# danshapero/sigma

Hardware: AMD Instinct MI355X
Metric: SpMV GB/s (achieved HBM) + CG iters/sec on 5-pt Laplacian, N=1e7 (higher is better)
Workload: dtype f64; 1 GPU; 5-point 2D Poisson CSR, 3162x3162 rows per GPU (rank 0: n=9998244, nnz=49978572), fp64 SpMV y=A*x; rows_per_gpu=9998244, nnz_per_gpu=49978572, parallelism=row-partition x1, matrix_resident_bytes_per_gpu=479920788, reference_layout_bytes_per_gpu=639735844, full=False

## Files before the change

sigma_amd/csrc/sgm_internal.hpp:

```cpp
#pragma once
#include <hip/hip_runtime.h>

#include <cstdarg>
#include <cstdint>
#include <cstdio>
#include <cstring>
#include <string>
#include <atomic>
#include <utility>
#include <vector>

#include "../../include/sigma_hip.h"

namespace sgm {

extern std::string g_err;
int fail(int code, const char *fmt, ...);

#define SGM_HIP(call)                                                              \
    do {                                                                           \
        hipError_t e__ = (call);                                                   \
        if (e__ != hipSuccess)                                                     \
            return sgm::fail(SGM_ERR_HIP, "%s:%d: %s -> %s", __FILE__, __LINE__,   \
                             #call, hipGetErrorString(e__));                       \
// ... 115 lines not shown
};

struct SliceSched { int32_t *tab = nullptr; int32_t lo = 0, hi = 0, grid = 0, iters = 0, band = 0; };

struct Part {
    MatOptions opt = g_opt.mat;
    int32_t n = 0;
    int32_t ncol_own = 0;
    int32_t n_halo = 0;
    int32_t int_lo = 0, int_hi = 0;
    int64_t nnz = 0;
    int64_t row_begin = 0;
    int32_t *rowptr = nullptr;
    int32_t *col = nullptr;
    double *val = nullptr;
    uint8_t *code = nullptr;
    int32_t *dict = nullptr;
    int32_t ndict = 0;
    int32_t dict_reach = 0;
    int32_t max_row = 0;
    double *sval = nullptr;
    uint32_t *scode = nullptr;
    int32_t *scol = nullptr;
    uint8_t *sbcode = nullptr;
    bool lean = false;
    double *sl_val = nullptr;
    int32_t *sl_col = nullptr;
    uint16_t *sl_perm = nullptr;
    int64_t *sl_off = nullptr;
    int64_t sl_total = 0;
    int32_t *sl_win0 = nullptr;
    int32_t sl_gs = 1;
    int32_t sl_span = 0;
    int32_t sw = 0;
    int32_t sched_period = 0;
    mutable SliceSched sched[3];
    mutable int nsched = 0;
    const int32_t *run_sched = nullptr;
    int32_t run_iters = 0;
    int32_t max_d = 0;
    int32_t *ecol = nullptr;
    double *eval = nullptr;
    int32_t *edeg = nullptr;
    uint8_t *ecode = nullptr;
    int32_t emdp = 0;
    int32_t *cb_perm = nullptr;
    double *cb_sval = nullptr;
    uint16_t *cb_lcol = nullptr;
    int32_t *cb_bstart = nullptr;
    uint16_t *cb_lpos = nullptr;
    void *cb_fdesc = nullptr;
    double *cb_P = nullptr;
    int32_t cb_cols = 0, cb_nb = 0, cb_R = 0, cb_ntiles = 0, cb_chunks = 0;
    int32_t cb_maxd = 0;
    int64_t cb_count = 0;
    double col_spread = -1.0;
    std::vector<HaloNbr> nbrs;
    double *xext = nullptr;
    int dot_grid_override = 0;
    int64_t xlen() const { return (int64_t)ncol_own + n_halo; }
};

}

namespace sgm { struct AlgPlan; void alg_plan_free(AlgPlan *p); void alg_plan_rows(const AlgPlan *p, int32_t out[2]); }

// ... 258 lines not shown
```

sigma_amd/csrc/sgm_layouts.hip:

```cpp
#include "sgm_spmv_select.hpp"

namespace sgm {

__global__ void k_dec1(int32_t *a, int64_t n)
{
    int64_t i = (int64_t)blockIdx.x * blockDim.x + threadIdx.x;
    const int64_t stride = (int64_t)gridDim.x * blockDim.x;
    for (; i < n; i += stride) a[i] -= 1;
}

__global__ void k_check_ptr1(const int32_t *__restrict__ ptr1, int64_t n, int64_t nnz, unsigned long long *bad)
{
    int64_t i = (int64_t)blockIdx.x * blockDim.x + threadIdx.x;
    const int64_t stride = (int64_t)gridDim.x * blockDim.x;
    for (; i <= n; i += stride) {
        const int32_t a = ptr1[i];
        bool ok = true;
        if (i == 0) ok = a == 1;
        if (i < n) ok = ok && ptr1[i + 1] >= a;
        else ok = ok && (int64_t)a - 1 == nnz;
        if (!ok) atomicMin(bad, (unsigned long long)i);
    }
}

// ... 245 lines not shown
{
    if (!p.lean || p.val) return SGM_OK;
    SGM_TRY(dalloc(&p.val, (size_t)p.nnz + 2));
    SGM_HIP(hipMemsetAsync(p.val + p.nnz, 0, 2 * sizeof(double), g_rt.stream));
    return SGM_OK;
}
void csr_release_arrays(const Part &cp)
{
    Part &p = const_cast<Part &>(cp);
    if (!p.lean || !lean_applies(p)) return;
    (void)hipStreamSynchronize(g_rt.stream);
    dfree(p.val); dfree(p.col); dfree(p.code);
    p.val = nullptr; p.col = nullptr; p.code = nullptr;
}

int pack_sliced(Part &p)
{
    if (p.sl_val && p.n > 0) {
        const int64_t nch = (((int64_t)p.n + kSlRows - 1) / kSlRows) * (kSlRows / kSellChunk);
        hipLaunchKernelGGL(k_sell_fill, dim3((unsigned)std::min<int64_t>((nch + 3) / 4, 65536)), dim3(256), 0, g_rt.stream, p.n,
                           (const int32_t *)p.rowptr, (const int32_t *)nullptr, (const double *)p.val, (const int64_t *)p.sl_off,
                           (const uint16_t *)p.sl_perm, (int32_t *)nullptr, p.sl_val);
        SGM_HIP(hipGetLastError());
    }
    if ((!p.scode && !p.scol && !p.sbcode) || p.n == 0) return SGM_OK;
    const int64_t nsl = ((int64_t)p.n + kSlRows - 1) / kSlRows;
    if (p.ecol)
        hipLaunchKernelGGL(k_sl_pack_ell, dim3((unsigned)std::min<int64_t>(nsl, 65536)), dim3(256), 0, g_rt.stream, p.n, p.sw,
                           p.max_d, (const double *)p.eval, p.sval);
    else
        hipLaunchKernelGGL(k_sl_pack, dim3((unsigned)std::min<int64_t>(nsl, 65536)), dim3(256), 0, g_rt.stream, p.n, p.sw,
                           (const int32_t *)p.rowptr, (const double *)p.val, p.sval);
    SGM_HIP(hipGetLastError());
    return SGM_OK;
}

__global__ void k_fill32(int64_t n, int32_t *a, int32_t v)
{
    int64_t i = (int64_t)blockIdx.x * blockDim.x + threadIdx.x;
    const int64_t stride = (int64_t)gridDim.x * blockDim.x;
    for (; i < n; i += stride) a[i] = v;
}

constexpr int kDictSlots = 1024;
constexpr int32_t kDictEmpty = INT32_MIN;
__global__ __launch_bounds__(256) void k_dict_collect(int32_t n, const int32_t *__restrict__ rowptr, const int32_t *__restrict__ col,
                                                      int32_t *table, int *count, int *max_row)
{
    constexpr int kLocal = 512;
    __shared__ int32_t ltab[kLocal];
    __shared__ int lcount;
    for (int t = threadIdx.x; t < kLocal; t += 256) ltab[t] = kDictEmpty;
    if (threadIdx.x == 0) lcount = 0;
    __syncthreads();
    int mr = 0;
    int32_t mine[8];
#pragma unroll
    for (int t = 0; t < 8; ++t) mine[t] = kDictEmpty;
    int next = 0;
    for (int32_t i = blockIdx.x * blockDim.x + threadIdx.x; i < n; i += gridDim.x * blockDim.x) {
        const int32_t s0 = rowptr[i], e = rowptr[i + 1];
        mr = max(mr, e - s0);
        for (int32_t k = s0; k < e; ++k) {
            const int32_t off = col[k] - i;
            bool known = false;
#pragma unroll
// ... 448 lines not shown
        return fail(SGM_ERR_UNSUPPORTED, "clone_csr_plain: single-GPU CSR matrices only");
    const Part &p = A->parts[0];
    SGM_TRY(csr_need_arrays(p));
    struct Release { const Part &p; ~Release() { csr_release_arrays(p); } } rel{p};
    sgm_mat C = new sgm_mat_s;
    C->fmt = SGM_FMT_CSR; C->nrow = A->nrow; C->ncol = A->ncol; C->nnz = A->nnz;
    C->parts.resize(1);
    Part &q = C->parts[0];
    q.opt.csr_offset_dict = 0; q.opt.csr_sliced = 0; q.opt.csr_sell = 0; q.opt.csr_lean = 0; q.opt.slice_sched = 0;
    q.n = p.n; q.ncol_own = p.ncol_own; q.n_halo = 0; q.nnz = p.nnz; q.max_row = p.max_row;
    hipStream_t st = g_rt.stream;
    int rc = dalloc(&q.rowptr, (size_t)p.n + 1);
    if (rc == SGM_OK) rc = dalloc(&q.col, (size_t)p.nnz + 4);
    if (rc == SGM_OK) rc = dalloc(&q.val, (size_t)p.nnz + 2);
    if (rc != SGM_OK) { sgm_mat_destroy(C); return rc; }
    (void)hipMemcpyAsync(q.rowptr, p.rowptr, ((size_t)p.n + 1) * 4, hipMemcpyDeviceToDevice, st);
    (void)hipMemsetAsync(q.col + p.nnz, 0, 16, st);
    (void)hipMemsetAsync(q.val + p.nnz, 0, 16, st);
    if (p.nnz) {
        (void)hipMemcpyAsync(q.col, p.col, (size_t)p.nnz * 4, hipMemcpyDeviceToDevice, st);
        (void)hipMemcpyAsync(q.val, p.val, (size_t)p.nnz * 8, hipMemcpyDeviceToDevice, st);
    }
    if (hipStreamSynchronize(st) != hipSuccess || hipGetLastError() != hipSuccess) { sgm_mat_destroy(C); return fail(SGM_ERR_HIP, "clone_csr_plain: copy failed"); }
    *out = C;
    return SGM_OK;
}

int rebuild_csr_formats(Part &p)
{
    SGM_TRY(csr_need_arrays(p));
    p.lean = false;
    dfree(p.code); dfree(p.dict); dfree(p.sval); dfree(p.scode); dfree(p.scol); dfree(p.sbcode);
    p.code = nullptr; p.dict = nullptr; p.sval = nullptr; p.scode = nullptr; p.scol = nullptr; p.sbcode = nullptr;
    free_sell(p);
    free_ell_colblock(p);
    p.ndict = 0; p.dict_reach = 0; p.sw = 0; p.max_row = 0; p.sched_period = 0;
    free_slice_sched(p);
    return build_offset_dict(p, nullptr, nullptr);
}
int rebuild_ell_formats(Part &p)
{
    dfree(p.ecode); dfree(p.dict); dfree(p.sval); dfree(p.scode);
    p.ecode = nullptr; p.dict = nullptr; p.dict_reach = 0; p.emdp = 0; p.sval = nullptr; p.scode = nullptr; p.sw = 0; p.sched_period = 0;
    free_slice_sched(p);
    SGM_TRY(build_ell_offset_dict(p));
    SGM_TRY(build_ell_colblock(p));
    return refresh_ell_colblock_values(p);
}
int sgm_invalidate_transpose(sgm_mat A)
{
    if (A->T) { sgm_mat_destroy(A->T); A->T = nullptr; }
    dfree(A->tperm);
    A->tperm = nullptr;
    A->t_stale = true;
    return SGM_OK;
}

void free_part(Part &p)
{
    dfree(p.rowptr); dfree(p.col); dfree(p.val); dfree(p.code); dfree(p.dict); dfree(p.sval); dfree(p.scode); dfree(p.scol); dfree(p.sbcode); dfree(p.ecol); dfree(p.eval); dfree(p.edeg); dfree(p.ecode); dfree(p.xext);
    for (auto &nb : p.nbrs) { dfree(nb.send_idx); dfree(nb.send_buf); }
    free_slice_sched(p);
    free_ell_colblock(p);
    free_sell(p);
    p = Part();
}

}
```

sigma_amd/csrc/sgm_mat.hip:

```cpp
#include "sgm_spmv_select.hpp"

namespace sgm {

int stage_in(Staged &s, const double *v, int64_t n, int where, bool copy)
{
    if (where == SGM_DEVICE && (reinterpret_cast<uintptr_t>(v) & 15) == 0) {
        s.dev = const_cast<double *>(v);
        return SGM_OK;
    }
    SGM_TRY(dalloc(&s.dev, (size_t)n));
    s.owned = true;
    if (copy)
        SGM_HIP(hipMemcpyAsync(s.dev, v, (size_t)n * 8,
                               where == SGM_HOST ? hipMemcpyHostToDevice : hipMemcpyDeviceToDevice,
                               g_rt.stream));
    return SGM_OK;
}
int stage_out(const Staged &s, double *v, int64_t n, int where)
{
    if (!s.owned) return SGM_OK;
    SGM_HIP(hipMemcpyAsync(v, s.dev, (size_t)n * 8,
                           where == SGM_HOST ? hipMemcpyDeviceToHost : hipMemcpyDeviceToDevice,
                           g_rt.stream));
    SGM_HIP(hipStreamSynchronize(g_rt.stream));
// ... 356 lines not shown
    return SGM_OK;
}

int sgm_mat_set_option(sgm_mat A, const char *name, int value)
{
    SGM_TRY(require_init());
    if (!A || !name) return fail(SGM_ERR_BAD_ARG, "sgm_mat_set_option: null argument");
    int v = 0;
    SGM_TRY(normalise_option(name, value, &v));
    MatOptions probe;
    if (!mat_option_field(probe, name)) return fail(SGM_ERR_BAD_ARG, "sgm_mat_set_option: '%s' is not a matrix option", name);
    if (A->fmt == SGM_FMT_COMPOSITE) {
        for (sgm_mat_s *B : A->blocks)
            if (B) SGM_TRY(sgm_mat_set_option(B, name, value));
        return SGM_OK;
    }
    const bool cb_shape = !strcmp(name, "ell_colblock_cols") || !strcmp(name, "ell_colblock_rows");
    for (Part &p : A->parts) {
        int *f = mat_option_field(p.opt, name);
        const int old = *f;
        *f = v;
        if (old == v) continue;
        if ((p.ecol || (!p.lean && p.rowptr && p.col && p.val && p.n_halo == 0 && !p.sval && !p.sl_val)) &&
            (cb_shape || (!strcmp(name, "ell_colblock") && ((old != 0) != (v != 0) || v == 2 || old == 2)))) {
            SGM_TRY(build_ell_colblock(p));
            SGM_TRY(refresh_ell_colblock_values(p));
            SGM_HIP(hipStreamSynchronize(g_rt.stream));
        }
        if (!strcmp(name, "csr_lean") && !p.ecol) {
            if (v == 0) { SGM_TRY(csr_need_arrays(p)); p.lean = false; }
            else csr_go_lean(p);
        }
        if (!strcmp(name, "slice_sched")) free_slice_sched(p);
    }
    if (A->T) SGM_TRY(sgm_mat_set_option(A->T, name, value));
    return SGM_OK;
}

int sgm_mat_matvec(sgm_mat A, const double *x, double *y, int where)
{
    return matvec_impl(A, x, y, where, false);
}

int sgm_mat_matvec_add(sgm_mat A, const double *x, double *y, int where)
{
    return matvec_impl(A, x, y, where, true);
}

int sgm_composite_create(sgm_mat *out, int32_t nrb, int32_t ncb, const int32_t *row_ptr, const int32_t *col_ptr,
                         const sgm_mat *blocks)
{
    SGM_TRY(require_init());
    if (!out || nrb < 1 || ncb < 1 || !row_ptr || !col_ptr || !blocks)
        return fail(SGM_ERR_BAD_ARG, "sgm_composite_create: bad argument");
    sgm_mat A = new sgm_mat_s;
    A->fmt = SGM_FMT_COMPOSITE;
    for (int i = 0; i <= nrb; ++i) A->blk_row_ptr.push_back(row_ptr[i] - 1);
    for (int j = 0; j <= ncb; ++j) A->blk_col_ptr.push_back(col_ptr[j] - 1);
    A->nrow = A->blk_row_ptr[nrb];
    A->ncol = A->blk_col_ptr[ncb];
    A->blocks.assign(blocks, blocks + (size_t)nrb * ncb);
    sgm_comm comm = nullptr;
    bool any_local = false;
    for (int it = 0; it < nrb; ++it)
        for (int jt = 0; jt < ncb; ++jt) {
            sgm_mat C = A->blocks[(size_t)it * ncb + jt];
// ... 142 lines not shown
    else if (use_sliced(p)) snprintf(name, len, "k_csr_sl<W=%d>", p.sw);
    else if (use_slicedb(p)) snprintf(name, len, "k_csr_slb<W=%d>", p.sw);
    else if (use_sliced32(p)) snprintf(name, len, "k_csr_sl32<W=%d>", p.sw);
    else if (use_sell(p)) snprintf(name, len, p.sl_win0 && p.opt.csr_xwindow ? "k_csr_sell<pad=%.3f,xw=%dx%d>" : "k_csr_sell<pad=%.3f>",
                                   p.nnz ? (double)p.sl_total / (double)p.nnz : 1.0, p.sl_span, p.sl_gs);
    else if (use_offset_dict(p)) snprintf(name, len, "k_csr_do<256,%d,CW=1>", do_tile_for(p));
    else if (use_row_owner(p)) snprintf(name, len, "k_csr_do<256,%d,CW=4>", do_tile_for(p));
    else if (use_row_lines(p)) snprintf(name, len, "k_csr_rl");
    else snprintf(name, len, "k_csr_spmv");
}
}
extern "C" {

int sgm_mat_kernel(sgm_mat A, char *buf, int len)
{
    if (!A || !buf || len < 1) return fail(SGM_ERR_BAD_ARG, "sgm_mat_kernel: bad argument");
    char name[64];
    if (A->fmt == SGM_FMT_COMPOSITE) snprintf(name, sizeof name, "composite");
    else part_kernel_name(A->parts[0], A->fmt, name, sizeof name);
    snprintf(buf, (size_t)len, "%s", name);
    return SGM_OK;
}

static int64_t part_resident_bytes(const Part &p)
{
    int64_t b = 0;
    const int64_t nsl = ((int64_t)p.n + kSlRows - 1) / kSlRows;
    if (p.rowptr) b += 4 * ((int64_t)p.n + 1);
    if (p.col) b += 4 * (p.nnz + 4);
    if (p.val) b += 8 * (p.nnz + 2);
    if (p.code) b += p.nnz + 16;
    if (p.dict) b += 4 * 256;
    if (p.sval) b += 8 * nsl * kSlRows * p.sw;
    if (p.scode) b += 4 * nsl * kSlRows;
    if (p.scol) b += 4 * nsl * kSlRows * p.sw;
    if (p.sbcode) b += nsl * kSlRows * ((p.sw + 7) / 8 * 8);
    if (p.sl_val) b += 12 * p.sl_total + 2 * nsl * kSlRows + 8 * (nsl * (kSlRows / kSellChunk) + 1);
    if (p.ecol) b += 4 * (int64_t)p.n * p.max_d;
    if (p.eval) b += 8 * (int64_t)p.n * p.max_d;
    if (p.edeg) b += 4 * (int64_t)p.n;
    if (p.ecode) b += (int64_t)p.n * p.emdp;
    if (p.xext) b += 8 * p.xlen();
    b += ell_colblock_resident_bytes(p);
    for (const auto &nb : p.nbrs) b += (int64_t)nb.send_count * (nb.send_buf ? 12 : 4);
    return b;
}
static int64_t part_matvec_bytes(const sgm_mat_s *A, const Part &p)
{
    const int64_t nsl = ((int64_t)p.n + kSlRows - 1) / kSlRows;
    int64_t m;
    if (A->fmt == SGM_FMT_ELL) {
        if (use_ell_colblock(p)) return ell_colblock_matvec_bytes(p);
        if (use_sliced_ell(p)) m = nsl * kSlRows * (8 * (int64_t)p.sw + 4);
        else if (p.ecode && p.opt.ell_offset_dict) m = (int64_t)p.n * (8 * (int64_t)p.max_d + p.emdp);
        else m = 12 * (int64_t)p.n * p.max_d;
    } else if (use_ell_colblock(p)) return ell_colblock_matvec_bytes(p);
    else if (use_sliced(p)) m = nsl * kSlRows * (8 * (int64_t)p.sw + 4);
    else if (use_slicedb(p)) m = nsl * kSlRows * (8 * (int64_t)p.sw + (p.sw + 7) / 8 * 8);
    else if (use_sliced32(p)) m = nsl * kSlRows * 12 * (int64_t)p.sw;
    else if (use_sell(p)) {
        m = 12 * p.sl_total + 2 * nsl * kSlRows + 8 * nsl * (kSlRows / kSellChunk);
        if (p.sl_win0 && p.opt.csr_xwindow)
            return m + ((nsl + p.sl_gs - 1) / p.sl_gs) * (8 * (int64_t)p.sl_span + 4) + 8 * (int64_t)p.n;
    }
    else if (use_offset_dict(p)) m = 9 * p.nnz + 4 * ((int64_t)p.n + 1);
    else m = 12 * p.nnz + 4 * ((int64_t)p.n + 1);
    return m + 8 * p.xlen() + 8 * (int64_t)p.n;
}

int sgm_mat_footprint(sgm_mat A, int64_t *resident_bytes, int64_t *matvec_bytes)
{
    if (!A) return fail(SGM_ERR_BAD_ARG, "sgm_mat_footprint: null matrix");
    int64_t res = 0, mv = 0;
    if (A->fmt == SGM_FMT_COMPOSITE) {
        for (sgm_mat C : A->blocks) {
            if (!C) continue;
            int64_t r = 0, m = 0;
            SGM_TRY(sgm_mat_footprint(C, &r, &m));
            mv += m + 8 * (int64_t)C->nrow;
        }
        mv += 8 * (int64_t)A->nrow;
    } else {
        for (const Part &p : A->parts) { res += part_resident_bytes(p); mv += part_matvec_bytes(A, p); }
        if (A->T) { int64_t r = 0; SGM_TRY(sgm_mat_footprint(A->T, &r, nullptr)); res += r + 4 * A->nnz; }
    }
    if (resident_bytes) *resident_bytes = res;
    if (matvec_bytes) *matvec_bytes = mv;
    return SGM_OK;
}
// ... 14 lines not shown
```

sigma_amd/csrc/sgm_runtime.hip:

```cpp
#include "sgm_internal.hpp"

#include <algorithm>

namespace sgm {

std::string g_err;
Runtime g_rt;
Options g_opt;
Heartbeat g_hb;

int fail(int code, const char *fmt, ...)
{
    char buf[1024];
    va_list ap;
    va_start(ap, fmt);
    vsnprintf(buf, sizeof buf, fmt, ap);
    va_end(ap);
    g_err = buf;
    return code;
}

bool trace_on()
{
    static const bool on = getenv("SGM_TRACE") != nullptr;
// ... 59 lines not shown
    SGM_HIP(hipStreamSynchronize(st));
    return SGM_OK;
}

#define SGM_OPT(group, field) if (!strcmp(name, #field)) return &o.field;
int *mat_option_field(MatOptions &o, const char *name)
{
    SGM_OPT(mat, csr_offset_dict) SGM_OPT(mat, ell_offset_dict) SGM_OPT(mat, csr_row_owner) SGM_OPT(mat, csr_row_lines)
    SGM_OPT(mat, csr_sliced) SGM_OPT(mat, csr_sell) SGM_OPT(mat, csr_xwindow) SGM_OPT(mat, csr_lean) SGM_OPT(mat, ell_colblock) SGM_OPT(mat, ell_colblock_cols)
    SGM_OPT(mat, ell_colblock_rows) SGM_OPT(mat, slice_sched) SGM_OPT(mat, coloring_pass)
    return nullptr;
}
int *solver_option_field(SolverOptions &o, const char *name)
{
    SGM_OPT(solver, cg_small) SGM_OPT(solver, bicgstab_small) SGM_OPT(solver, krylov_graph) SGM_OPT(solver, dot_order)
    SGM_OPT(solver, gmres_cgs2) SGM_OPT(solver, dist_halo_fused) SGM_OPT(solver, coop_spin_limit) SGM_OPT(solver, cg_coop_variant)
    SGM_OPT(solver, reorder_solve)
    return nullptr;
}
int *pc_option_field(PcOptions &o, const char *name)
{
    SGM_OPT(pc, ildu_strips) SGM_OPT(pc, ildu_rows) SGM_OPT(pc, pipeline_spin_limit) SGM_OPT(pc, ildu_reorder)
    return nullptr;
}
#undef SGM_OPT

int normalise_option(const char *name, int value, int *out)
{
    int v = value;
    if (!strcmp(name, "ell_colblock_cols")) v = std::min(kEllcbMaxCols, std::max(2, value)) & ~1;
    else if (!strcmp(name, "ell_colblock_rows")) v = value == 512 ? 512 : value == 256 ? 256 : 0;
    else if (!strcmp(name, "ildu_reorder")) v = value != 0;
    else if (!strcmp(name, "csr_sell")) v = value < 0 ? 0 : value > 2 ? 2 : value;
    else if (!strcmp(name, "csr_lean") || !strcmp(name, "csr_xwindow")) v = value != 0;
    else if (!strcmp(name, "slice_sched")) v = value <= 0 ? 0 : value == 1 ? 1 : std::max(4, value);
    else if (!strcmp(name, "krylov_graph")) v = value <= 0 ? 0 : value == 1 ? 1 : std::max(16, (value + 15) / 16 * 16);
    else if (!strcmp(name, "cg_small")) v = std::max(0, value);
    else if (!strcmp(name, "dist_halo_fused") || !strcmp(name, "reorder_solve")) v = value < 0 ? 0 : value > 2 ? 2 : value;
    else if (!strcmp(name, "coop_spin_limit")) v = std::max(0, value);
    else if (!strcmp(name, "gmres_cgs2")) v = value != 0;
    else if (!strcmp(name, "cg_coop_variant")) {
        const int r = value & 15;
        if (value < 0 || value > 31 || (r != 0 && r != 1 && r != 2 && r != 4 && r != 8))
            return fail(SGM_ERR_BAD_ARG, "option cg_coop_variant: rows per thread 0 (by size), 1, 2, 4 or 8, + 16 = no one-XCD variant");
    }
    else if (!strcmp(name, "coloring_pass")) v = value < 0 ? 0 : value > 2 ? 2 : value;
    else if (!strcmp(name, "pipeline_spin_limit")) v = std::max(0, value);
    else if (!strcmp(name, "dot_order") && value != 0 && value != 1)
        return fail(SGM_ERR_BAD_ARG, "option dot_order is 0 (tree) or 1 (the reference's sequential order)");
    *out = v;
    return SGM_OK;
}

}

using namespace sgm;

extern "C" {

int sgm_init(int device)
{
    int count = 0;
    hipError_t e = hipGetDeviceCount(&count);
    if (e != hipSuccess || count <= 0)
        return fail(SGM_ERR_NO_DEVICE,
                    "sgm_init: no HIP device visible (%s); this library has no CPU path",
// ... 110 lines not shown
```

sigma_amd/csrc/sgm_spmv.hip:

```cpp
#include "sgm_spmv_select.hpp"
#include "sgm_plan_host.hpp"

namespace sgm {




__device__ inline int64_t rowblock_of(int it, int b, int grid, int64_t nrb = 0, int mode = 1)
{
    const int per = grid >> 3;
    if (mode == 2) {
        const int64_t chunk = (nrb + 7) / 8;
        const int64_t local = (int64_t)it * per + (b >> 3);
        return local < chunk ? (int64_t)(b & 7) * chunk + local : nrb;
    }
    return (int64_t)it * grid + (int64_t)(b & 7) * per + (b >> 3);
}


template <class T>
__device__ inline T ld_stream(const T *p, bool nt)
{
    return nt ? __builtin_nontemporal_load(p) : *p;
}
// ... 319 lines not shown
            while (k < kend) {
                const int cnt = min(kend - k, U);
                double xv[U], vv[U];
#pragma unroll
                for (int u = 0; u < U; ++u)
                    if (u < cnt) {
                        const int o = k + u - ts;
                        xv[u] = CW == 1 ? x[row + dl[cl[o]]] : x[(int32_t)cl4[o]];
                        vv[u] = vl[o];
                    }
#pragma unroll
                for (int u = 0; u < U; ++u)
                    if (u < cnt) z = z + vv[u] * xv[u];
                k += cnt;
            }
        }
        if (row < n) {
            const double yi = ADD ? (chain ? z : y0 + z) : 0.0 + z;
            __builtin_nontemporal_store(yi, y + row);
            if (DOT_W) dwy += w[row] * yi;
            if (DOT_YY) dyy += yi * yi;
        }
    }
    if (DOT_W) {
        const double t = block_sum<BLOCK>(dwy, red);
        if (tid == 0) part_wy[blockIdx.x] = t;
    }
    if (DOT_YY) {
        const double t = block_sum<BLOCK>(dyy, red);
        if (tid == 0) part_yy[blockIdx.x] = t;
    }
}

template <int W, bool ADD, bool DOT_W, bool DOT_YY>
__global__ __launch_bounds__(256) void k_csr_sl(
    int32_t n, const uint32_t *__restrict__ scode, const int32_t *__restrict__ dict,
    const double *__restrict__ sval, const double *__restrict__ x, double *__restrict__ y,
    const double *__restrict__ w, double *__restrict__ part_wy, double *__restrict__ part_yy,
    const int *__restrict__ flag_done, int gen, int remap, const int32_t *__restrict__ sched, int sched_iters)
{
    constexpr int BLOCK = 256;
    __shared__ int32_t dl[16];
    __shared__ double red[BLOCK / 64];
    const int st = flag_done ? *flag_done : 0;
    const int tid = threadIdx.x;
    const bool chain = (remap & 256) != 0;
    const int32_t dv = tid < 16 ? dict[tid] : 0;
    const int64_t nsl = ((int64_t)n + kSlRows - 1) / kSlRows;
    double dwy = 0.0, dyy = 0.0;

    int64_t first = blockIdx.x;
    if ((remap & 255) >= 3) {
        const int G = (remap & 255) == 3 ? 8 : (remap & 255) == 4 ? 2 : (remap & 255) == 6 ? 64 : (remap & 255) == 7 ? 128 : 32;
        const int xcd = blockIdx.x & 7, loc = blockIdx.x >> 3;
        first = (int64_t)(loc / G) * (8 * G) + xcd * G + loc % G;
    }
    int64_t sl = sched ? sched[blockIdx.x] : first;
    int sit = 0;
    u32x2 cw = {0xffffffffu, 0xffffffffu};
    f64x2 v[W];
    auto load_slice = [&](int64_t s_) {
        const int32_t row_ = (int32_t)(s_ * kSlRows) + 2 * tid;
        cw = __builtin_nontemporal_load(reinterpret_cast<const u32x2 *>(scode + row_));
        const f64x2 *vb = reinterpret_cast<const f64x2 *>(sval + s_ * (int64_t)(W * kSlRows)) + tid;
#pragma unroll
        for (int u = 0; u < W; ++u) v[u] = __builtin_nontemporal_load(vb + u * BLOCK);
    };
    bool have = sl >= 0 && sl < nsl;
    if (have) load_slice(sl);
    if (st && gen >= st) return;
    if (tid < 16) dl[tid] = dv;
    __syncthreads();
    while (have) {
        int64_t nxt = sl + gridDim.x;
        if (sched) { ++sit; nxt = sit < sched_iters ? sched[(int64_t)sit * gridDim.x + blockIdx.x] : -1; }
        const int32_t row = (int32_t)(sl * kSlRows) + 2 * tid;
        f64x2 y0 = {0.0, 0.0};
        if (ADD) {
            if (row + 1 < n) y0 = *reinterpret_cast<const f64x2 *>(y + row);
            else if (row < n) y0.x = y[row];
        }
        double xa[W], xb[W];
#pragma unroll
        for (int u = 0; u < W; ++u) {
            const uint32_t ca = (cw.x >> (4 * u)) & 15u, cb = (cw.y >> (4 * u)) & 15u;
            xa[u] = ca != 15u ? x[row + dl[ca]] : 0.0;
            xb[u] = cb != 15u ? x[row + 1 + dl[cb]] : 0.0;
        }
        f64x2 z;
        z.x = (ADD && chain) ? y0.x : 0.0;
        z.y = (ADD && chain) ? y0.y : 0.0;
#pragma unroll
        for (int u = 0; u < W; ++u) {
            if (((cw.x >> (4 * u)) & 15u) != 15u) z.x = z.x + v[u].x * xa[u];
            if (((cw.y >> (4 * u)) & 15u) != 15u) z.y = z.y + v[u].y * xb[u];
        }
        f64x2 yi;
        yi.x = ADD ? (chain ? z.x : y0.x + z.x) : 0.0 + z.x;
        yi.y = ADD ? (chain ? z.y : y0.y + z.y) : 0.0 + z.y;
        if (row + 1 < n) {
            __builtin_nontemporal_store(yi, reinterpret_cast<f64x2 *>(y + row));
            if (DOT_W) { const f64x2 wv = *reinterpret_cast<const f64x2 *>(w + row); dwy += wv.x * yi.x; dwy += wv.y * yi.y; }
            if (DOT_YY) { dyy += yi.x * yi.x; dyy += yi.y * yi.y; }
        } else if (row < n) {
            __builtin_nontemporal_store(yi.x, y + row);
            if (DOT_W) dwy += w[row] * yi.x;
            if (DOT_YY) dyy += yi.x * yi.x;
        }
        sl = nxt;
        have = sl >= 0 && sl < nsl;
        if (have) load_slice(sl);
    }
    if (DOT_W) {
        const double t = block_sum<BLOCK>(dwy, red);
        if (tid == 0) part_wy[blockIdx.x] = t;
    }
    if (DOT_YY) {
        const double t = block_sum<BLOCK>(dyy, red);
        if (tid == 0) part_yy[blockIdx.x] = t;
    }
}

template <bool ADD, bool DOT_W, bool DOT_YY, bool XW = false, int GS = 1>
__global__ __launch_bounds__(256 * GS) void k_csr_sell(
    int32_t n, const int64_t *__restrict__ off, const uint16_t *__restrict__ perm, const int32_t *__restrict__ scol,
    const double *__restrict__ sval, const double *__restrict__ x, double *__restrict__ y, const double *__restrict__ w,
    double *__restrict__ part_wy, double *__restrict__ part_yy, const int *__restrict__ flag_done, int gen, int remap,
    const int32_t *__restrict__ win0 = nullptr, int32_t span = 0, int32_t xlen = 0)
{
    constexpr int BLOCK = 256 * GS;
    extern __shared__ double xs[];
    __shared__ double red[BLOCK / 64];
    const int st = flag_done ? *flag_done : 0;
    const int lane = threadIdx.x & 63;
    const int wave = __builtin_amdgcn_readfirstlane(threadIdx.x >> 6);
    const bool chain = (remap & 256) != 0;
    const int64_t nsl = ((int64_t)n + kSlRows - 1) / kSlRows;
    double dwy = 0.0, dyy = 0.0;
    if (st && gen >= st) return;

    int64_t first = blockIdx.x;
    if ((remap & 255) >= 3) {
        const int G = (remap & 255) == 3 ? 8 : (remap & 255) == 4 ? 2 : (remap & 255) == 6 ? 64 : (remap & 255) == 7 ? 128 : 32;
        const int xcd = blockIdx.x & 7, loc = blockIdx.x >> 3;
// ... 433 lines not shown
    const bool dict = use_offset_dict(p);
#define L(B, T, DW, DY)                                                                                 \
    do {                                                                                                \
        if (dict)                                                                                       \
            hipLaunchKernelGGL((k_csr_do<B, T, 1, ADD, DW, DY>), dim3(grid), dim3(B), 0, st, p.n, p.rowptr, \
                               p.code, p.dict, p.val, x, y, w, pwy, pyy, flag, gen, c.remap | g_launch_flags); \
        else                                                                                            \
            hipLaunchKernelGGL((k_csr_do<B, T, 4, ADD, DW, DY>), dim3(grid), dim3(B), 0, st, p.n, p.rowptr, \
                               reinterpret_cast<const uint8_t *>(p.col), p.dict, p.val, x, y, w, pwy, pyy, flag, \
                               gen, c.remap | g_launch_flags);                                          \
    } while (0)
#define LV(B, T)                                \
    if (c.block == B && tile == T) {            \
        if (w && pyy) L(B, T, true, true);      \
        else if (w) L(B, T, true, false);       \
        else if (pyy) L(B, T, false, true);     \
        else L(B, T, false, false);             \
        return;                                 \
    }
    SGM_DO_VARIANTS(LV)
#undef LV
#undef L
}

template <bool ADD>
static void launch_csr_sl(const Part &p, int grid, const double *x, double *y, const double *w,
                          double *pwy, double *pyy, const int *flag, int gen)
{
    const SpmvCfg &c = spmv_cfg();
    hipStream_t st = g_rt.stream;
    int mode = c.remap == 1 ? ((grid <= kMaxGrid / 2 || (int64_t)p.n < (int64_t)32768 * kSlRows) ? 5 : 0) : (c.remap >= 3 ? c.remap : 0);
    if (mode >= 3 && grid % (8 * (mode == 3 ? 8 : mode == 4 ? 2 : mode == 6 ? 64 : mode == 7 ? 128 : 32)) != 0) mode = 0;
#define L(WW, DW, DY)                                                                                   \
    hipLaunchKernelGGL((k_csr_sl<WW, ADD, DW, DY>), dim3(grid), dim3(256), 0, st, p.n, p.scode, p.dict, \
                       p.sval, x, y, w, pwy, pyy, flag, gen, mode | g_launch_flags, p.run_sched, p.run_iters)
#define LV(WW)                                \
    if (p.sw == WW) {                         \
        if (w && pyy) L(WW, true, true);      \
        else if (w) L(WW, true, false);       \
        else if (pyy) L(WW, false, true);     \
        else L(WW, false, false);             \
        return;                               \
    }
    SGM_SL_WIDTHS(LV)
#undef LV
#undef L
}

template <bool ADD>
static void launch_csr_sl32(const Part &p, int grid, const double *x, double *y, const double *w,
                            double *pwy, double *pyy, const int *flag, int gen)
{
    hipStream_t st = g_rt.stream;
    const SpmvCfg &c = spmv_cfg();
    int mode = c.remap == 1 ? ((grid <= kMaxGrid / 2 || (int64_t)p.n < (int64_t)32768 * kSlRows) ? 5 : 0) : (c.remap >= 3 ? c.remap : 0);
    if (mode >= 3 && grid % (8 * (mode == 3 ? 8 : mode == 4 ? 2 : mode == 6 ? 64 : mode == 7 ? 128 : 32)) != 0) mode = 0;
#define L(WW, DW, DY)                                                                                     \
    hipLaunchKernelGGL((k_csr_sl32<WW, ADD, DW, DY>), dim3(grid), dim3(256), 0, st, p.n, p.scol, p.sval, x, y, \
                       w, pwy, pyy, flag, gen, mode | g_launch_flags)
#define LV(WW)                                \
    if (p.sw == WW) {                         \
        if (w && pyy) L(WW, true, true);      \
        else if (w) L(WW, true, false);       \
        else if (pyy) L(WW, false, true);     \
        else L(WW, false, false);             \
        return;                               \
    }
    SGM_SL32_WIDTHS(LV)
// ... 177 lines not shown
    for (int i = 0; i < p.nsched; ++i)
        if (p.sched[i].lo == lo && p.sched[i].hi == hi && p.sched[i].grid == grid) return p.sched[i].tab ? &p.sched[i] : nullptr;
    if (p.nsched >= 3) return nullptr;
    SliceSched &ss = p.sched[p.nsched++];
    ss.lo = lo; ss.hi = hi; ss.grid = grid; ss.tab = nullptr; ss.band = band;
    std::vector<int32_t> tab;
    int iters = 0;
    slice_sched_table(nsl, p.sched_period, grid, band, tab, iters);
    int32_t *d = nullptr;
    if (dalloc(&d, tab.size()) != SGM_OK) return nullptr;
    if (hipMemcpy(d, tab.data(), tab.size() * sizeof(int32_t), hipMemcpyHostToDevice) != hipSuccess) { dfree(d); return nullptr; }
    ss.tab = d; ss.iters = iters;
    return &ss;
}
void free_slice_sched(Part &p)
{
    for (int i = 0; i < p.nsched; ++i) { dfree(p.sched[i].tab); p.sched[i] = SliceSched(); }
    p.nsched = 0;
}

static void launch_range(sgm_mat A, const Part &p, const RowRange &r, const double *x, double *y, bool add,
                         const double *w, double *pwy, double *pyy, const int *flag_done, int gen)
{
    Part v;
    v.opt = p.opt;
    v.n = r.hi - r.lo;
    v.nnz = (int64_t)((double)p.nnz * v.n / (p.n > 0 ? p.n : 1));
    v.n_halo = p.n_halo; v.ncol_own = p.ncol_own;
    v.rowptr = p.rowptr + r.lo; v.col = p.col; v.val = p.val; v.code = p.code; v.dict = p.dict;
    v.max_row = p.max_row;
    const bool sliced = use_sliced(p), slicedb = !sliced && use_slicedb(p), sliced32 = !sliced && !slicedb && use_sliced32(p);
    if (sliced || slicedb)
        if (const SliceSched *ss = slice_sched(p, r.lo, r.hi, r.grid)) { v.run_sched = ss->tab; v.run_iters = ss->iters; }
    if (sliced) { v.sval = p.sval + (int64_t)r.lo * p.sw; v.scode = p.scode + r.lo; v.sw = p.sw; }
    if (slicedb) { v.sval = p.sval + (int64_t)r.lo * p.sw; v.sbcode = p.sbcode + (int64_t)r.lo * ((p.sw + 7) / 8 * 8); v.sw = p.sw; }
    if (sliced32) { v.sval = p.sval + (int64_t)r.lo * p.sw; v.scol = p.scol + (int64_t)r.lo * p.sw; v.sw = p.sw; }
    const bool sell = !sliced && !slicedb && !sliced32 && use_sell(p);
    if (sell) {
        v.sl_val = p.sl_val; v.sl_col = p.sl_col;
        v.sl_off = p.sl_off + r.lo / kSellChunk; v.sl_perm = p.sl_perm + r.lo;
        v.sl_gs = p.sl_gs;
        v.sl_win0 = p.sl_win0 ? p.sl_win0 + r.lo / (kSlRows * p.sl_gs) : nullptr; v.sl_span = p.sl_span;
    }
    const bool dict = use_offset_dict(p);
    const double *xs = dict ? x + r.lo : x;
    double *ys = y + r.lo;
    const double *ws = w ? w + r.lo : nullptr;
    double *pw = pwy ? pwy + r.part_off : nullptr, *py = pyy ? pyy + r.part_off : nullptr;
    if (sliced) {
        if (add) launch_csr_sl<true>(v, r.grid, xs, ys, ws, pw, py, flag_done, gen);
        else launch_csr_sl<false>(v, r.grid, xs, ys, ws, pw, py, flag_done, gen);
    } else if (slicedb) {
        if (add) launch_csr_slb<true>(v, r.grid, xs, ys, ws, pw, py, flag_done, gen);
        else launch_csr_slb<false>(v, r.grid, xs, ys, ws, pw, py, flag_done, gen);
    } else if (sliced32) {
        if (add) launch_csr_sl32<true>(v, r.grid, x, ys, ws, pw, py, flag_done, gen);
        else launch_csr_sl32<false>(v, r.grid, x, ys, ws, pw, py, flag_done, gen);
    } else if (sell) {
        if (add) launch_csr_sell<true>(v, r.grid, x, ys, ws, pw, py, flag_done, gen);
        else launch_csr_sell<false>(v, r.grid, x, ys, ws, pw, py, flag_done, gen);
    } else if (use_row_owner(p)) {
        if (add) launch_csr_do<true>(v, r.grid, xs, ys, ws, pw, py, flag_done, gen);
        else launch_csr_do<false>(v, r.grid, xs, ys, ws, pw, py, flag_done, gen);
    } else if (use_row_lines(p)) {
        if (add) launch_csr_rl<true>(v, r.grid, xs, ys, ws, pw, py, flag_done, gen);
        else launch_csr_rl<false>(v, r.grid, xs, ys, ws, pw, py, flag_done, gen);
    } else {
// ... 153 lines not shown
```

sigma_amd/csrc/sgm_spmv_select.hpp:

```cpp
#pragma once
#include "sgm_internal.hpp"

#include <type_traits>

#include <hipcub/hipcub.hpp>

#include <algorithm>
#include <cstdlib>
#include <string>
#include <vector>

namespace sgm {

typedef double f64x2 __attribute__((ext_vector_type(2)));
typedef int i32x2 __attribute__((ext_vector_type(2)));
typedef int i32x4 __attribute__((ext_vector_type(4)));
typedef uint32_t u32x2 __attribute__((ext_vector_type(2)));
typedef uint16_t u16x2 __attribute__((ext_vector_type(2)));
typedef unsigned int u32x4s __attribute__((ext_vector_type(4)));
#define SGM_SLB_WIDTHS(X) X(9) X(12) X(15) X(16) X(19) X(20) X(24) X(25) X(27) X(28) X(32)
#define SGM_SL_WIDTHS(X) X(3) X(5) X(7) X(8)
#define SGM_SL32_WIDTHS(X) X(3) X(5) X(7) X(8) X(12) X(16) X(20) X(24) X(28) X(32)
constexpr int kSlRows = 512;
constexpr int kSellChunk = 128;
// ... 4 lines not shown


struct SpmvCfg { int block = 256, vpt = 2, nt = 1, maxgrid = 0, remap = 1, do_vpt = 0; };
static SpmvCfg &spmv_cfg()
{
    static SpmvCfg c;
    static bool init = false;
    if (!init) {
        init = true;
        if (c.maxgrid > kMaxGrid) c.maxgrid = kMaxGrid;
        if (c.block != 256 && c.block != 512 && c.block != 1024) c.block = 256;
        if (c.vpt != 2 && c.vpt != 4 && c.vpt != 8) c.vpt = 2;
        if (c.block == 1024 && c.vpt == 8) c.vpt = 4;
    }
    return c;
}

int resident_per_cu(bool dict, int block, int v, int cw = 4);
static const SliceSched *slice_sched(const Part &p, int32_t lo, int32_t hi, int grid);
void free_slice_sched(Part &p);
int ell_grid(const Part &p);
bool use_ell_colblock(const Part &p);
int ell_colblock_grid(const Part &p);
int build_ell_colblock(Part &p);
int refresh_ell_colblock_values(Part &p);
void free_ell_colblock(Part &p);
int launch_ell_colblock(const Part &p, int grid, const double *x, double *y, bool add, bool chain, const double *w,
                        double *pwy, double *pyy, const int *flag, int gen);
int64_t ell_colblock_resident_bytes(const Part &p);
int64_t ell_colblock_matvec_bytes(const Part &p);
static bool do_block_ok() { const int b = spmv_cfg().block; return b == 256 || b == 512; }
static bool use_offset_dict(const Part &p) { return (p.code || (p.lean && p.dict)) && p.opt.csr_offset_dict && do_block_ok(); }
static bool use_sliced(const Part &p) { return p.scode && p.opt.csr_sliced && p.opt.csr_offset_dict; }
static bool use_sliced32(const Part &p) { return p.scol && p.opt.csr_sliced && !p.ecol; }
static bool use_slicedb(const Part &p) { return p.sbcode && p.opt.csr_sliced && p.opt.csr_offset_dict; }
static bool use_sell(const Part &p) { return p.sl_val && p.opt.csr_sliced && p.opt.csr_sell && !p.ecol; }
static bool any_sliced(const Part &p) { return use_sliced(p) || use_sliced32(p) || use_slicedb(p) || use_sell(p); }
static bool use_sliced_ell(const Part &p) { return p.ecol && p.scode && p.opt.csr_sliced && p.opt.ell_offset_dict; }
static bool use_row_owner(const Part &p)
{
    return use_offset_dict(p) || (do_block_ok() && p.opt.csr_row_owner && p.max_row > 0 && p.max_row <= 64);
}

static bool use_row_lines(const Part &p)
{
    return p.opt.csr_row_lines && !any_sliced(p) && !use_row_owner(p) && p.n > 0 && p.max_row <= 4096 &&
           p.nnz >= 16 * (int64_t)p.n && (int64_t)p.max_row * p.n <= 4 * p.nnz;
}
int row_lines_resident_per_cu();

#define SGM_DO_VARIANTS(X) X(256, 1024) X(256, 1536) X(256, 1920) X(256, 2048) X(256, 4096) X(512, 2048) X(512, 3072) X(512, 3840)
static int do_tile_for(const Part &p)
{
    const SpmvCfg &c = spmv_cfg();
    static const int t256[] = {1024, 1536, 1920, 2048, 4096}, t512[] = {2048, 3072, 3840};
    const int *tiles = c.block == 512 ? t512 : t256;
    const int nt = c.block == 512 ? 3 : (use_offset_dict(p) ? 4 : 5);
    if (c.do_vpt) return tiles[std::min(std::max(c.do_vpt - 1, 0), nt - 1)];
    const double per_block = (double)p.nnz / (p.n > 0 ? p.n : 1) * c.block + 4;
    for (int i = 0; i < nt; ++i)
        if (per_block <= tiles[i]) return tiles[i];
    return tiles[nt - 1];
}

static int grid_for_rows(const Part &p, int64_t rows, int64_t limit, bool dots = true)
{
// ... 12 lines not shown
    return (int)g;
}

struct RowRange { int32_t lo, hi; int grid, part_off; };
static int spmv_ranges(const Part &p, RowRange out[3], bool dots = true, bool whole = false)
{
    int nr = 0, off = 0;
    auto add = [&](int32_t lo, int32_t hi) {
        if (hi <= lo) return;
        out[nr] = RowRange{lo, hi, grid_for_rows(p, hi - lo, nr == 0 ? kMaxGrid / 4 : kMaxGrid / 8), off};
        off += out[nr].grid;
        ++nr;
    };
    if (p.n_halo == 0 || p.int_hi <= p.int_lo || whole) {
        if (any_sliced(p)) {
            out[0] = RowRange{0, p.n, grid_for_rows(p, p.n > 0 ? p.n : 1, kMaxGrid, dots), 0};
            return 1;
        }
        add(0, p.n > 0 ? p.n : 1);
        if (nr) out[0].hi = p.n;
        return nr;
    }
    add(p.int_lo, p.int_hi);
    add(0, p.int_lo);
    add(p.int_hi, p.n);
    return nr;
}


void free_part(Part &p);
void csr_go_lean(Part &p);
int lean_val_buffer(Part &p);
int pack_sliced(Part &p);
int build_ell_offset_dict(Part &p);
__global__ void k_ell_transpose(const int32_t *__restrict__ node, const double *__restrict__ val, int32_t *__restrict__ ecol,
                                double *__restrict__ eval, int32_t n, int32_t max_d, int32_t ncol = 0, unsigned long long *bad = nullptr);
}
```

Measured before the change: 6285 GB/s.

## Replace streamed sliced-CSR values with a per-offset value table when uniform

```diff
diff --git a/sigma_amd/csrc/sgm_internal.hpp b/sigma_amd/csrc/sgm_internal.hpp
--- a/sigma_amd/csrc/sgm_internal.hpp
+++ b/sigma_amd/csrc/sgm_internal.hpp
@@ -171,6 +171,7 @@
     int32_t *sl_win0 = nullptr;
     int32_t sl_gs = 1;
     int32_t sl_span = 0;
+    double *vtab = nullptr;
     int32_t sw = 0;
     int32_t sched_period = 0;
     mutable SliceSched sched[3];
diff --git a/sigma_amd/csrc/sgm_layouts.hip b/sigma_amd/csrc/sgm_layouts.hip
--- a/sigma_amd/csrc/sgm_layouts.hip
+++ b/sigma_amd/csrc/sgm_layouts.hip
@@ -301,6 +301,72 @@
         hipLaunchKernelGGL(k_sl_pack, dim3((unsigned)std::min<int64_t>(nsl, 65536)), dim3(256), 0, g_rt.stream, p.n, p.sw,
                            (const int32_t *)p.rowptr, (const double *)p.val, p.sval);
     SGM_HIP(hipGetLastError());
+    return refresh_value_table(p);
+}
+
+__global__ __launch_bounds__(256) void k_vtab_claim(int64_t rows_padded, int W, const uint32_t *__restrict__ scode,
+                                                    const unsigned long long *__restrict__ sval, unsigned int *claimed,
+                                                    unsigned long long *tab)
+{
+    __shared__ unsigned int lc[16];
+    if (threadIdx.x < 16) lc[threadIdx.x] = claimed[threadIdx.x];
+    __syncthreads();
+    for (int64_t r = (int64_t)blockIdx.x * 256 + threadIdx.x; r < rows_padded; r += (int64_t)gridDim.x * 256) {
+        const uint32_t cw = scode[r];
+        if (cw == 0xffffffffu) continue;
+        for (int u = 0; u < W; ++u) {
+            const uint32_t c = (cw >> (4 * u)) & 15u;
+            if (c == 15u || lc[c]) continue;
+            if (atomicExch(&lc[c], 1u) != 0u) continue;
+            if (atomicCAS(&claimed[c], 0u, 1u) != 0u) continue;
+            tab[c] = sval[((r >> 9) * W + u) * kSlRows + (r & (kSlRows - 1))];
+        }
+    }
+}
+__global__ __launch_bounds__(256) void k_vtab_verify(int64_t rows_padded, int W, const uint32_t *__restrict__ scode,
+                                                     const unsigned long long *__restrict__ sval,
+                                                     const unsigned long long *__restrict__ tab, unsigned int *differs)
+{
+    __shared__ unsigned long long tl[16];
+    if (threadIdx.x < 16) tl[threadIdx.x] = tab[threadIdx.x];
+    __syncthreads();
+    bool diff = false;
+    for (int64_t r = (int64_t)blockIdx.x * 256 + threadIdx.x; r < rows_padded; r += (int64_t)gridDim.x * 256) {
+        const uint32_t cw = scode[r];
+        if (cw == 0xffffffffu) continue;
+        for (int u = 0; u < W; ++u) {
+            const uint32_t c = (cw >> (4 * u)) & 15u;
+            if (c != 15u && sval[((r >> 9) * W + u) * kSlRows + (r & (kSlRows - 1))] != tl[c]) diff = true;
+        }
+    }
+    if (diff) atomicOr(differs, 1u);
+}
+static_assert(kSlRows == 512, "the checks above index slices with r >> 9");
+int refresh_value_table(Part &p)
+{
+    if (!value_table_wanted(p)) { dfree(p.vtab); p.vtab = nullptr; return SGM_OK; }
+    hipStream_t st = g_rt.stream;
+    const int64_t rows_padded = (((int64_t)p.n + kSlRows - 1) / kSlRows) * kSlRows;
+    unsigned int *scr = nullptr;
+    SGM_TRY(dalloc(&scr, 17));
+    if (!p.vtab) { const int rc = dalloc(&p.vtab, 16); if (rc != SGM_OK) { dfree(scr); p.vtab = nullptr; return rc; } }
+    unsigned int differs = 1;
+    hipError_t e = hipMemsetAsync(scr, 0, 17 * sizeof(unsigned int), st);
+    if (e == hipSuccess) e = hipMemsetAsync(p.vtab, 0, 16 * sizeof(double), st);
+    if (e == hipSuccess) {
+        const unsigned grid = (unsigned)std::min<int64_t>(rows_padded / 256, 4096);
+        hipLaunchKernelGGL(k_vtab_claim, dim3(grid), dim3(256), 0, st, rows_padded, (int)p.sw, (const uint32_t *)p.scode,
+                           reinterpret_cast<const unsigned long long *>(p.sval), scr, reinterpret_cast<unsigned long long *>(p.vtab));
+        hipLaunchKernelGGL(k_vtab_verify, dim3(grid), dim3(256), 0, st, rows_padded, (int)p.sw, (const uint32_t *)p.scode,
+                           reinterpret_cast<const unsigned long long *>(p.sval),
+                           reinterpret_cast<const unsigned long long *>(p.vtab), scr + 16);
+        e = hipGetLastError();
+    }
+    if (e == hipSuccess) e = hipMemcpyAsync(&differs, scr + 16, sizeof differs, hipMemcpyDeviceToHost, st);
+    if (e == hipSuccess) e = hipStreamSynchronize(st);
+    dfree(scr);
+    if (e != hipSuccess || differs) { dfree(p.vtab); p.vtab = nullptr; }
+    if (e != hipSuccess) return fail(SGM_ERR_HIP, "value table check: %s", hipGetErrorString(e));
     return SGM_OK;
 }
 
@@ -815,6 +881,7 @@
     p.lean = false;
     dfree(p.code); dfree(p.dict); dfree(p.sval); dfree(p.scode); dfree(p.scol); dfree(p.sbcode);
     p.code = nullptr; p.dict = nullptr; p.sval = nullptr; p.scode = nullptr; p.scol = nullptr; p.sbcode = nullptr;
+    dfree(p.vtab); p.vtab = nullptr;
     free_sell(p);
     free_ell_colblock(p);
     p.ndict = 0; p.dict_reach = 0; p.sw = 0; p.max_row = 0; p.sched_period = 0;
@@ -841,7 +908,7 @@
 
 void free_part(Part &p)
 {
-    dfree(p.rowptr); dfree(p.col); dfree(p.val); dfree(p.code); dfree(p.dict); dfree(p.sval); dfree(p.scode); dfree(p.scol); dfree(p.sbcode); dfree(p.ecol); dfree(p.eval); dfree(p.edeg); dfree(p.ecode); dfree(p.xext);
+    dfree(p.rowptr); dfree(p.col); dfree(p.val); dfree(p.code); dfree(p.dict); dfree(p.sval); dfree(p.scode); dfree(p.scol); dfree(p.sbcode); dfree(p.ecol); dfree(p.eval); dfree(p.edeg); dfree(p.ecode); dfree(p.xext); dfree(p.vtab);
     for (auto &nb : p.nbrs) { dfree(nb.send_idx); dfree(nb.send_buf); }
     free_slice_sched(p);
     free_ell_colblock(p);
diff --git a/sigma_amd/csrc/sgm_mat.hip b/sigma_amd/csrc/sgm_mat.hip
--- a/sigma_amd/csrc/sgm_mat.hip
+++ b/sigma_amd/csrc/sgm_mat.hip
@@ -412,6 +412,7 @@
             else csr_go_lean(p);
         }
         if (!strcmp(name, "slice_sched")) free_slice_sched(p);
+        if (!strcmp(name, "csr_sliced")) SGM_TRY(refresh_value_table(p));
     }
     if (A->T) SGM_TRY(sgm_mat_set_option(A->T, name, value));
     return SGM_OK;
@@ -620,6 +621,7 @@
     if (p.code) b += p.nnz + 16;
     if (p.dict) b += 4 * 256;
     if (p.sval) b += 8 * nsl * kSlRows * p.sw;
+    if (p.vtab) b += 128;
     if (p.scode) b += 4 * nsl * kSlRows;
     if (p.scol) b += 4 * nsl * kSlRows * p.sw;
     if (p.sbcode) b += nsl * kSlRows * ((p.sw + 7) / 8 * 8);
@@ -643,6 +645,7 @@
         else if (p.ecode && p.opt.ell_offset_dict) m = (int64_t)p.n * (8 * (int64_t)p.max_d + p.emdp);
         else m = 12 * (int64_t)p.n * p.max_d;
     } else if (use_ell_colblock(p)) return ell_colblock_matvec_bytes(p);
+    else if (use_value_table(p)) m = nsl * kSlRows * 4 + 128;
     else if (use_sliced(p)) m = nsl * kSlRows * (8 * (int64_t)p.sw + 4);
     else if (use_slicedb(p)) m = nsl * kSlRows * (8 * (int64_t)p.sw + (p.sw + 7) / 8 * 8);
     else if (use_sliced32(p)) m = nsl * kSlRows * 12 * (int64_t)p.sw;
diff --git a/sigma_amd/csrc/sgm_runtime.hip b/sigma_amd/csrc/sgm_runtime.hip
--- a/sigma_amd/csrc/sgm_runtime.hip
+++ b/sigma_amd/csrc/sgm_runtime.hip
@@ -115,6 +115,7 @@
     else if (!strcmp(name, "ell_colblock_rows")) v = value == 512 ? 512 : value == 256 ? 256 : 0;
     else if (!strcmp(name, "ildu_reorder")) v = value != 0;
     else if (!strcmp(name, "csr_sell")) v = value < 0 ? 0 : value > 2 ? 2 : value;
+    else if (!strcmp(name, "csr_sliced")) v = value < 0 ? 0 : value > 3 ? 3 : value;
     else if (!strcmp(name, "csr_lean") || !strcmp(name, "csr_xwindow")) v = value != 0;
     else if (!strcmp(name, "slice_sched")) v = value <= 0 ? 0 : value == 1 ? 1 : std::max(4, value);
     else if (!strcmp(name, "krylov_graph")) v = value <= 0 ? 0 : value == 1 ? 1 : std::max(16, (value + 15) / 16 * 16);
diff --git a/sigma_amd/csrc/sgm_spmv.hip b/sigma_amd/csrc/sgm_spmv.hip
--- a/sigma_amd/csrc/sgm_spmv.hip
+++ b/sigma_amd/csrc/sgm_spmv.hip
@@ -375,20 +375,23 @@
     }
 }
 
-template <int W, bool ADD, bool DOT_W, bool DOT_YY>
+template <int W, bool ADD, bool DOT_W, bool DOT_YY, bool TAB = false>
 __global__ __launch_bounds__(256) void k_csr_sl(
     int32_t n, const uint32_t *__restrict__ scode, const int32_t *__restrict__ dict,
     const double *__restrict__ sval, const double *__restrict__ x, double *__restrict__ y,
     const double *__restrict__ w, double *__restrict__ part_wy, double *__restrict__ part_yy,
-    const int *__restrict__ flag_done, int gen, int remap, const int32_t *__restrict__ sched, int sched_iters)
+    const int *__restrict__ flag_done, int gen, int remap, const int32_t *__restrict__ sched, int sched_iters,
+    const double *__restrict__ vtab = nullptr)
 {
     constexpr int BLOCK = 256;
     __shared__ int32_t dl[16];
+    __shared__ double tl[TAB ? 16 : 1];
     __shared__ double red[BLOCK / 64];
     const int st = flag_done ? *flag_done : 0;
     const int tid = threadIdx.x;
     const bool chain = (remap & 256) != 0;
     const int32_t dv = tid < 16 ? dict[tid] : 0;
+    const double tv = (TAB && tid < 16) ? vtab[tid] : 0.0;
     const int64_t nsl = ((int64_t)n + kSlRows - 1) / kSlRows;
     double dwy = 0.0, dyy = 0.0;
 
@@ -401,22 +404,36 @@
     int64_t sl = sched ? sched[blockIdx.x] : first;
     int sit = 0;
     u32x2 cw = {0xffffffffu, 0xffffffffu};
-    f64x2 v[W];
+    f64x2 v[TAB ? 1 : W];
     auto load_slice = [&](int64_t s_) {
         const int32_t row_ = (int32_t)(s_ * kSlRows) + 2 * tid;
         cw = __builtin_nontemporal_load(reinterpret_cast<const u32x2 *>(scode + row_));
-        const f64x2 *vb = reinterpret_cast<const f64x2 *>(sval + s_ * (int64_t)(W * kSlRows)) + tid;
-#pragma unroll
-        for (int u = 0; u < W; ++u) v[u] = __builtin_nontemporal_load(vb + u * BLOCK);
+        if (!TAB) {
+            const f64x2 *vb = reinterpret_cast<const f64x2 *>(sval + s_ * (int64_t)(W * kSlRows)) + tid;
+#pragma unroll
+            for (int u = 0; u < W; ++u) v[u] = __builtin_nontemporal_load(vb + u * BLOCK);
+        }
+    };
+    auto after = [&](int64_t s_) -> int64_t {
+        if (sched) { ++sit; return sit < sched_iters ? sched[(int64_t)sit * gridDim.x + blockIdx.x] : -1; }
+        return s_ + gridDim.x;
+    };
+    auto load_codes = [&](int64_t s_) -> u32x2 {
+        u32x2 c = {0xffffffffu, 0xffffffffu};
+        if (s_ >= 0 && s_ < nsl) c = __builtin_nontemporal_load(reinterpret_cast<const u32x2 *>(scode + (int32_t)(s_ * kSlRows) + 2 * tid));
+        return c;
     };
     bool have = sl >= 0 && sl < nsl;
+    int64_t s1 = -1;
+    u32x2 cw1 = {0xffffffffu, 0xffffffffu};
     if (have) load_slice(sl);
+    if (TAB && have) { s1 = after(sl); cw1 = load_codes(s1); }
     if (st && gen >= st) return;
     if (tid < 16) dl[tid] = dv;
+    if (TAB && tid < 16) tl[tid] = tv;
     __syncthreads();
     while (have) {
-        int64_t nxt = sl + gridDim.x;
-        if (sched) { ++sit; nxt = sit < sched_iters ? sched[(int64_t)sit * gridDim.x + blockIdx.x] : -1; }
+        const int64_t nxt = TAB ? s1 : after(sl);
         const int32_t row = (int32_t)(sl * kSlRows) + 2 * tid;
         f64x2 y0 = {0.0, 0.0};
         if (ADD) {
@@ -424,19 +441,23 @@
             else if (row < n) y0.x = y[row];
         }
         double xa[W], xb[W];
+        f64x2 tvv[TAB ? W : 1];
 #pragma unroll
         for (int u = 0; u < W; ++u) {
             const uint32_t ca = (cw.x >> (4 * u)) & 15u, cb = (cw.y >> (4 * u)) & 15u;
             xa[u] = ca != 15u ? x[row + dl[ca]] : 0.0;
             xb[u] = cb != 15u ? x[row + 1 + dl[cb]] : 0.0;
-        }
+            if (TAB) { tvv[u].x = tl[ca]; tvv[u].y = tl[cb]; }
+        }
+        u32x2 cw2 = {0xffffffffu, 0xffffffffu};
+        if (TAB) { s1 = after(s1); cw2 = load_codes(s1); }
         f64x2 z;
         z.x = (ADD && chain) ? y0.x : 0.0;
         z.y = (ADD && chain) ? y0.y : 0.0;
 #pragma unroll
         for (int u = 0; u < W; ++u) {
-            if (((cw.x >> (4 * u)) & 15u) != 15u) z.x = z.x + v[u].x * xa[u];
-            if (((cw.y >> (4 * u)) & 15u) != 15u) z.y = z.y + v[u].y * xb[u];
+            if (((cw.x >> (4 * u)) & 15u) != 15u) z.x = z.x + (TAB ? tvv[u].x : v[u].x) * xa[u];
+            if (((cw.y >> (4 * u)) & 15u) != 15u) z.y = z.y + (TAB ? tvv[u].y : v[u].y) * xb[u];
         }
         f64x2 yi;
         yi.x = ADD ? (chain ? z.x : y0.x + z.x) : 0.0 + z.x;
@@ -452,7 +473,8 @@
         }
         sl = nxt;
         have = sl >= 0 && sl < nsl;
-        if (have) load_slice(sl);
+        if (TAB) { cw = cw1; cw1 = cw2; }
+        else if (have) load_slice(sl);
     }
     if (DOT_W) {
         const double t = block_sum<BLOCK>(dwy, red);
@@ -952,8 +974,16 @@
     int mode = c.remap == 1 ? ((grid <= kMaxGrid / 2 || (int64_t)p.n < (int64_t)32768 * kSlRows) ? 5 : 0) : (c.remap >= 3 ? c.remap : 0);
     if (mode >= 3 && grid % (8 * (mode == 3 ? 8 : mode == 4 ? 2 : mode == 6 ? 64 : mode == 7 ? 128 : 32)) != 0) mode = 0;
 #define L(WW, DW, DY)                                                                                   \
-    hipLaunchKernelGGL((k_csr_sl<WW, ADD, DW, DY>), dim3(grid), dim3(256), 0, st, p.n, p.scode, p.dict, \
-                       p.sval, x, y, w, pwy, pyy, flag, gen, mode | g_launch_flags, p.run_sched, p.run_iters)
+    do {                                                                                                \
+        if (p.vtab)                                                                                     \
+            hipLaunchKernelGGL((k_csr_sl<WW, ADD, DW, DY, true>), dim3(grid), dim3(256), 0, st, p.n, p.scode, p.dict, \
+                               p.sval, x, y, w, pwy, pyy, flag, gen, mode | g_launch_flags, p.run_sched, p.run_iters, \
+                               (const double *)p.vtab);                                                 \
+        else                                                                                            \
+            hipLaunchKernelGGL((k_csr_sl<WW, ADD, DW, DY, false>), dim3(grid), dim3(256), 0, st, p.n, p.scode, p.dict, \
+                               p.sval, x, y, w, pwy, pyy, flag, gen, mode | g_launch_flags, p.run_sched, p.run_iters, \
+                               (const double *)nullptr);                                                \
+    } while (0)
 #define LV(WW)                                \
     if (p.sw == WW) {                         \
         if (w && pyy) L(WW, true, true);      \
@@ -1197,7 +1227,7 @@
     const bool sliced = use_sliced(p), slicedb = !sliced && use_slicedb(p), sliced32 = !sliced && !slicedb && use_sliced32(p);
     if (sliced || slicedb)
         if (const SliceSched *ss = slice_sched(p, r.lo, r.hi, r.grid)) { v.run_sched = ss->tab; v.run_iters = ss->iters; }
-    if (sliced) { v.sval = p.sval + (int64_t)r.lo * p.sw; v.scode = p.scode + r.lo; v.sw = p.sw; }
+    if (sliced) { v.sval = p.sval + (int64_t)r.lo * p.sw; v.scode = p.scode + r.lo; v.sw = p.sw; v.vtab = use_value_table(p) ? p.vtab : nullptr; }
     if (slicedb) { v.sval = p.sval + (int64_t)r.lo * p.sw; v.sbcode = p.sbcode + (int64_t)r.lo * ((p.sw + 7) / 8 * 8); v.sw = p.sw; }
     if (sliced32) { v.sval = p.sval + (int64_t)r.lo * p.sw; v.scol = p.scol + (int64_t)r.lo * p.sw; v.sw = p.sw; }
     const bool sell = !sliced && !slicedb && !sliced32 && use_sell(p);
diff --git a/sigma_amd/csrc/sgm_spmv_select.hpp b/sigma_amd/csrc/sgm_spmv_select.hpp
--- a/sigma_amd/csrc/sgm_spmv_select.hpp
+++ b/sigma_amd/csrc/sgm_spmv_select.hpp
@@ -60,6 +60,14 @@
 static bool do_block_ok() { const int b = spmv_cfg().block; return b == 256 || b == 512; }
 static bool use_offset_dict(const Part &p) { return (p.code || (p.lean && p.dict)) && p.opt.csr_offset_dict && do_block_ok(); }
 static bool use_sliced(const Part &p) { return p.scode && p.opt.csr_sliced && p.opt.csr_offset_dict; }
+constexpr int64_t kValueTableMinBytes = (int64_t)32 << 20;
+static bool value_table_wanted(const Part &p)
+{
+    if (p.opt.csr_sliced < 1 || p.opt.csr_sliced > 2 || p.ecol || !p.scode || !p.sval || !p.dict || p.sw > 8 || p.n_halo != 0 || p.n < 1) return false;
+    const int64_t nsl = ((int64_t)p.n + kSlRows - 1) / kSlRows;
+    return p.opt.csr_sliced == 2 || 8 * nsl * kSlRows * p.sw >= kValueTableMinBytes;
+}
+static bool use_value_table(const Part &p) { return p.vtab && use_sliced(p) && value_table_wanted(p); }
 static bool use_sliced32(const Part &p) { return p.scol && p.opt.csr_sliced && !p.ecol; }
 static bool use_slicedb(const Part &p) { return p.sbcode && p.opt.csr_sliced && p.opt.csr_offset_dict; }
 static bool use_sell(const Part &p) { return p.sl_val && p.opt.csr_sliced && p.opt.csr_sell && !p.ecol; }
@@ -138,6 +146,7 @@
 void csr_go_lean(Part &p);
 int lean_val_buffer(Part &p);
 int pack_sliced(Part &p);
+int refresh_value_table(Part &p);
 int build_ell_offset_dict(Part &p);
 __global__ void k_ell_transpose(const int32_t *__restrict__ node, const double *__restrict__ val, int32_t *__restrict__ ecol,
                                 double *__restrict__ eval, int32_t n, int32_t max_d, int32_t ncol = 0, unsigned long long *bad = nullptr);
```

Result: slower. 4335 GB/s (-31.0%).
